# CaNS-World/CaLES

Measured on AMD Instinct MI355X. Metric: time-steps/sec, higher is better.
Workload: dtype f64; 1 GPU; turbulent channel 512x512x512, sgstype=dsmag, PP/PP/NN pressure BCs, bulk forcing in x (BASELINE.json configs[2]); 3 RK substeps/step; decomposition=single GPU

## Files before the change

cales_amd/csrc/common.hpp:

```cpp
#pragma once
#include <hip/hip_runtime.h>
#include <cstdint>
#include <cstdio>
#include <cstdlib>
#include <cstring>
#include <cmath>
#include <string>
#include <vector>
#include "../../include/cales.h"

typedef cales_real real;
#ifdef CALES_SINGLE
typedef float2 real2;
#define CALES_EPS 1.1920929e-07f
#define CALES_BIG 3.4028235e38f
#else
typedef double2 real2;
#define CALES_EPS 2.220446049250313e-16
#define CALES_BIG 1.7976931348623157e308
#endif
constexpr int RSZ = (int)sizeof(real);
constexpr int LINE_REALS = 128 / RSZ;
__host__ __device__ inline real2 make_real2(real x, real y) { real2 r; r.x = x; r.y = y; return r; }

// ... 13 lines not shown
  __host__ __device__ inline real at(int i, int j, int n1) const {
    const real bcv = bc[i + (size_t)(n1 + 2) * j];
    real r = 0.;
    if (cf == 'c') { if (ctype == 'D') r = -2. * bcv / dlc / dlf; else if (ctype == 'N') r = sgn * bcv / dlf; }
    else           { if (ctype == 'D') r = -bcv / dlc / dlf;      else if (ctype == 'N') r = sgn * bcv / dlc; }
    return r * alpha;
  }
};

struct Comm {
  cales_halo_cb halo = nullptr; cales_alltoall_cb a2a = nullptr; cales_allreduce_cb allred = nullptr; void *user = nullptr;
  real *A = nullptr, *B = nullptr; int64_t nbuf = 0;
  bool on = false;
  cales_halo_s_cb halo_s = nullptr; cales_alltoall_part_cb a2a_part = nullptr;
  bool halo_second_stream = false, a2a_second_stream = false, has_lo = false, has_hi = false;
};

struct Spec {
  int blocked, cw, n2l, n3;
  int nyq = 0;
  __host__ __device__ inline size_t at_slab(const Geom &g, int m, int jl, int k) const {
    if (!blocked) return (g.ix(0, jl, k) >> 1) + (size_t)m;
    const int peer = m / cw, mm = m - peer * cw;
    return (size_t)mm + (size_t)cw * ((size_t)(jl - 1) + (size_t)n2l * ((size_t)(k - 1) + (size_t)n3 * peer));
  }
  __host__ __device__ inline size_t at_mode(const Geom &g, int mm, int j, int k) const {
    if (!blocked) return (g.ix(0, j, k) >> 1) + (size_t)mm;
    const int peer = (j - 1) / n2l, jl = (j - 1) - peer * n2l;
    return (size_t)mm + (size_t)cw * ((size_t)jl + (size_t)n2l * ((size_t)(k - 1) + (size_t)n3 * peer));
  }
};

struct Flags {
  bool unfolded_correc = false, unfolded_mom = false, eager_projection = false, lazy_projection = false, helmholtz_z_per_column = false, unfused_imp_rhs = false, unfused_correc = false, unfused_forcing = false, unfused_fillps = false, unfused_mean = false, keep_last_rhs = false, wide_offsets = false, dsmag_reference_sequence = false, dsmag_xghosts = false, smag_reference_sequence = false, gaussel_march = false, fft_generic = false, fft_no_odd_radix = false, keep_null_mode = false, unfused_rk = false, overlap = false, xghosts_in_step = false, unmerged_bc = false, no_nyquist_packing = false, sgs_six_components = false;
  int kchunk = 0; long tile_min_blocks = 2048;
  std::string test_bad_launch;
  void read_env() {
    test_bad_launch = getenv("CALES_TEST_BAD_LAUNCH") ? getenv("CALES_TEST_BAD_LAUNCH") : "";
    unfolded_mom = getenv("CALES_UNFOLDED_MOM") != nullptr;
    lazy_projection = getenv("CALES_LAZY_PROJECTION") != nullptr;
    eager_projection = getenv("CALES_EAGER_PROJECTION") != nullptr;
    unfolded_correc = getenv("CALES_UNFOLDED_CORREC") != nullptr;
    helmholtz_z_per_column = getenv("CALES_HELMHOLTZ_Z_PER_COLUMN") != nullptr;
    unfused_imp_rhs = getenv("CALES_UNFUSED_IMP_RHS") != nullptr;
    unfused_correc = getenv("CALES_UNFUSED_CORREC") != nullptr;
    unfused_forcing = getenv("CALES_UNFUSED_FORCING") != nullptr;
    unfused_fillps = getenv("CALES_UNFUSED_FILLPS") != nullptr;
    unfused_mean = getenv("CALES_UNFUSED_MEAN") != nullptr;
    keep_last_rhs = getenv("CALES_KEEP_LAST_RHS") != nullptr;
    wide_offsets = getenv("CALES_WIDE_OFFSETS") != nullptr;
    dsmag_reference_sequence = getenv("CALES_DSMAG_REFERENCE_SEQUENCE") != nullptr;
    dsmag_xghosts = getenv("CALES_DSMAG_XGHOSTS") != nullptr;
    sgs_six_components = getenv("CALES_SGS_SIX_COMPONENTS") != nullptr;
    smag_reference_sequence = getenv("CALES_SMAG_REFERENCE_SEQUENCE") != nullptr;
    gaussel_march = getenv("CALES_GAUSSEL_MARCH") != nullptr;
    no_nyquist_packing = getenv("CALES_NO_NYQUIST_PACKING") != nullptr;
    fft_generic = getenv("CALES_FFT_GENERIC") != nullptr;
    fft_no_odd_radix = getenv("CALES_FFT_NO_ODD_RADIX") != nullptr;
    xghosts_in_step = getenv("CALES_XGHOSTS_IN_STEP") != nullptr;
    keep_null_mode = getenv("CALES_KEEP_NULL_MODE") != nullptr;
    unfused_rk = getenv("CALES_UNFUSED_RK") != nullptr;
    overlap = getenv("CALES_OVERLAP") != nullptr && atoi(getenv("CALES_OVERLAP")) != 0 && getenv("CALES_NO_OVERLAP") == nullptr;
    unmerged_bc = getenv("CALES_UNMERGED_BC") != nullptr;
    kchunk = getenv("CALES_KCHUNK") ? atoi(getenv("CALES_KCHUNK")) : 0;
    tile_min_blocks = getenv("CALES_TILE_MIN_BLOCKS") ? atol(getenv("CALES_TILE_MIN_BLOCKS")) : 2048;
  }
};

struct StepPlan {
  bool valid = false;
  bool in_visct_zero = false, in_sgs_first = false;
  bool xskip = false;
  bool fold_correc = false;
  bool fold_rows2 = false;
  bool fold_mom = false;
  bool lazy_last = false;
  bool defer_imp_rhs = false;
  bool any_wm = false, skip_first_wm = false;
  bool fuse_cu = false;
  bool defer_force = false;
  bool fuse_fill = false;
  bool visct_ghosts = false;
  bool keep_last_rhs = false;
  int mean_mask = 0, force_mask = 0;
};

struct BandMap { int gx, gy, gz, sub; };
struct TileGeom { dim3 block, grid; int kchunk = 0; BandMap bm{0, 0, 0, 0}; };
// ... 362 lines not shown
```

cales_amd/csrc/k_solver.hip:

```cpp
#include "common.hpp"

struct __attribute__((aligned(2 * sizeof(real)))) cpx { real x, y; };
__device__ inline cpx cadd(cpx a, cpx b) { return {a.x + b.x, a.y + b.y}; }
__device__ inline cpx csub(cpx a, cpx b) { return {a.x - b.x, a.y - b.y}; }
__device__ inline cpx cmul(cpx a, cpx b) { return {a.x * b.x - a.y * b.y, a.x * b.y + a.y * b.x}; }
__device__ inline cpx cconj(cpx a) { return {a.x, -a.y}; }
template <int INV> __device__ inline cpx mul_mi(cpx a) { return INV ? cpx{-a.y, a.x} : cpx{a.y, -a.x}; }

template <int R, int INV>
__device__ inline void fft_stage(const cpx *__restrict__ in, cpx *__restrict__ out, int N, int Ns, int t, int T, const cpx *__restrict__ tw) {
  const int M = N / R, tstep = N / (Ns * R);
  for (int j = t; j < M; j += T) {
    const int k = j % Ns;
    cpx v[R];
#pragma unroll
    for (int r = 0; r < R; ++r) v[r] = in[j + r * M];
    if (Ns > 1) {
#pragma unroll
      for (int r = 1; r < R; ++r) { cpx w = tw[k * r * tstep]; if (INV) w.y = -w.y; v[r] = cmul(v[r], w); }
    }
    const int j0 = (j - k) * R + k;
    if (R == 2) {
      out[j0] = cadd(v[0], v[1]); out[j0 + Ns] = csub(v[0], v[1]);
    } else if (R == 4) {
// ... 1118 lines not shown
      if (ch == 0) sp = 0.;
      real xv = rprev[q] - V[M - 2] * sp - cp[M - 2] * s;
      real mine = (rL == M - 2) ? xv : s;
      col[q * P + M - 2] = xv;
#pragma unroll
      for (int r = M - 3; r >= 0; --r) { xv = col[q * P + r] - V[r] * sp - cp[r] * xv; col[q * P + r] = xv; if (PER && r == rL) mine = xv; }
      col[q * P + M - 1] = s;
      if (PER) {
        const real p11 = __shfl(xv, 0, 64), p1n = __shfl(mine, cL, 64);
        const real an = ra[nz - 1], bn = rb_[nz - 1], cn = rc[nz - 1];
        const real den = (bn + lam) + cn * e1 + an * eL + CALES_EPS;
        const real pn = nullc ? 0. : ((pnr[q] - cn * p11) - an * p1n) * (1. / den);
#pragma unroll
        for (int r = 0; r < M - 1; ++r) if (k0 + r < nsys) col[q * P + r] = col[q * P + r] + E[r] * pn;
        if (k0 + M - 1 < nsys) col[q * P + M - 1] = s + Es * pn;
        if (ch == nsys / M) col[q * P + nsys % M] = pn;
      }
    }
  }
  __syncthreads();
  {
    constexpr int W2 = W / 2, KP2 = NT / W2, NQ2 = 64 * M / KP2;
    const int x = 2 * (t % W2), kk = t / W2;
    const bool ok = W * tile + x < ndbl;
    size_t o = base + x + (size_t)kk * kst;
    int kq = kk;
    asm volatile("" : "+v"(o), "+v"(kq));
    const size_t step = (size_t)KP2 * kst;
#pragma unroll
    for (int q = 0; q < NQ2; ++q) {
      const int k = kq + KP2 * q;
      if (ok && k < nz) *reinterpret_cast<real2 *>(p + o) = make_real2(shz[x * P + k + k / M], shz[(x + 1) * P + k + k / M]);
      o += step;
    }
  }
}
template <int M, int HERM>
__global__ __launch_bounds__(256) void k_gaussel_nyq(Geom g, int nz, int N, int nh, real lscale, const real *__restrict__ abc, const real *__restrict__ lamx,
                                                     const real *__restrict__ lamy, real2 *__restrict__ p, int fixnull, Spec S,
                                                     const real *__restrict__ ra = nullptr, const real *__restrict__ rb_ = nullptr, const real *__restrict__ rc = nullptr) {
  extern __shared__ real shz[];
  constexpr int NV = 1, PER = 0, CP = M + 1, P = 64 * CP + GT_PAD, NT = 256;
  constexpr bool TL = false;
  const real *tabl = nullptr;
  const int nsys = nz;
  const int t = threadIdx.x, ky = HERM ? blockIdx.x : 2 * blockIdx.x, kp = HERM ? (N - ky) % N : ky + 1;
  for (int k = t; k < 64 * M; k += NT) {
    real2 z1 = make_real2(0., 0.), z2 = z1;
    if (k < nz) { z1 = p[S.at_mode(g, 0, ky + 1, k + 1)]; z2 = p[S.at_mode(g, 0, kp + 1, k + 1)]; }
    const int o = k + k / M;
    if (HERM) {
      shz[0 * P + o] = 0.5 * (z1.x + z2.x); shz[1 * P + o] = 0.5 * (z1.y - z2.y);
      shz[2 * P + o] = 0.5 * (z1.y + z2.y); shz[3 * P + o] = -0.5 * (z1.x - z2.x);
    } else { shz[0 * P + o] = z1.x; shz[1 * P + o] = z1.y; shz[2 * P + o] = z2.x; shz[3 * P + o] = z2.y; }
  }
  __syncthreads();
  const int x = t >> 6, ch = t & 63;
  const bool colok = true;
  if (colok) {
    const real lam = HERM ? (lamx[x < 2 ? 0 : nh] + lamy[ky]) * lscale : (lamx[(x & 1) ? nh : 0] + lamy[x < 2 ? ky : kp]) * lscale;
    const bool nullc = fixnull && lam == 0.;
    real *col = shz + x * P + ch * CP;
    const int k0 = ch * M;
    real cp[M - 1], V[M - 1];
    real cprev = 0., vprev = 0., rprev[NV] = {};
    real pnr[NV] = {}, E[PER ? M - 1 : 1] = {}, eprev = 0.;
// ... 389 lines not shown

enum class XKernel { fft_x8, fft_x4, dst1, fft_x };
enum class YKernel { fft_y16, fft_y8, fft_y8r, fft_y4, dst1, fft_y };
enum class ZKernel { herm, tile, ri, periodic_real, periodic_cpx };
static bool radix8_y(YKernel k) { return k == YKernel::fft_y16 || k == YKernel::fft_y8 || k == YKernel::fft_y8r; }
typedef void (*FftX8)(Geom, int, int, const cpx *, const cpx *, const cpx *, real *, real, Spec, real2 *, FillArgs, long, long);
typedef void (*FftX4)(Geom, FftPlan, int, const cpx *, const cpx *, real *, real, Spec, real2 *);
typedef void (*FftX)(Geom, FftPlan, int, int, const cpx *, const cpx *, const cpx *, real *, real, Spec, real2 *);
typedef void (*Dst1)(Geom, FftPlan, int, const cpx *, real *, real, Spec, real2 *, int, int);
typedef void (*FftY16)(Geom, int, int, const cpx *, const cpx *, Spec, real2 *, int, int);
typedef void (*FftY8)(Geom, int, int, int, const cpx *, const cpx *, Spec, real2 *, int, int);
typedef void (*FftY8r)(Geom, int, int, int, const cpx *, Spec, real2 *, int, int);
typedef void (*FftY4)(Geom, FftPlan, int, int, const cpx *, const cpx *, Spec, real2 *);
typedef void (*FftY)(Geom, FftPlan, int, int, int, const cpx *, const cpx *, Spec, real2 *);
struct XPass {
  XKernel k = XKernel::fft_x;
  union { FftX8 x8[3]; FftX4 x4[2]; FftX x[2]; Dst1 dst1[2]; } fn = {{nullptr, nullptr, nullptr}};
  int threads = 256, rows = 1; size_t lds = 0;
  int odd = 0;
  FftPlan plan;
  const cpx *tw = nullptr, *twp = nullptr, *twd = nullptr;
};
struct YPass {
  YKernel k = YKernel::fft_y;
  union { FftY16 y16[2]; FftY8 y8[2]; FftY8r y8r[2]; FftY4 y4[2]; FftY y[2]; Dst1 dst1[2]; } fn = {{nullptr, nullptr}};
  int threads = 256, cols = 1; size_t lds = 0;
  int odd = 0;
  FftPlan plan;
  const cpx *tw = nullptr, *twd = nullptr;
};
constexpr int tile_m(int nz) { return nz <= 128 ? 2 : nz <= 256 ? 4 : nz <= 512 ? 8 : 16; }
static bool tile_takes(const cales_ctx *c, int nz, bool periodic) { return nz >= (periodic ? 4 : 2) && nz <= 1024 && !c->fl.gaussel_march; }
constexpr int TILE_TAB = 3 * 64 * 16;
struct ZTile { int M = 0, NV = 0, PER = 0, DUD = 0, ndbl = 0, nrow = 0; bool persistent = false; real *tab = nullptr; };
struct SolvePath {
  int xkind = 0, ykind = 0;
  XPass xp; YPass yp; ZKernel zk = ZKernel::ri;
  int nz = 0; bool periodic_z = false, poisson = false;
  ZTile zt;
  int fixnull = 0;
  bool refnull = false;
  bool null_switch = false;
  bool nyq = false;
  int cw = 0;
  real *lamx = nullptr, *lamy = nullptr; real normfft = 1.;
};
struct SolveSched {
  real2 *slab_spec = nullptr, *mode_spec = nullptr;
  int nch = 1, kpc = 0; long rows = 0;
  unsigned xblk_f = 0, xblk_b = 0; int xit_f = 1, xit_b = 1, ykc = 1;
  int ncol = 0, ncol_y = 0, mofs = 0, nmodes = 0;
  int64_t a2a_stride = 0, a2a_chunk = 0; int npart = 0;
  Spec S; TileMap T{}; dim3 gz;
};
static real2 *spec_of(real2 *staged, real *pp) { return staged ? staged : reinterpret_cast<real2 *>(pp + 1); }
enum class HzForm { thomas_periodic, thomas_per_column, tile, cols };
struct HzPath {
  HzForm form = HzForm::cols; int nz = 0, q = 0; ZTile zt; TileMap T{};
  real alpha[4] = {0., 0., 0., 0.}; bool ok[4] = {false, false, false, false}; int next = 0;
};
struct Solver {
  real *twx = nullptr, *twx_post = nullptr, *twy = nullptr, *twy_post = nullptr, *twyd = nullptr;
  real *tw4x = nullptr, *tw4y = nullptr, *twy4 = nullptr;
  SolvePath pres, vel[3]; SolveSched sched_pres, sched_vel[3];
  real *d_mpart = nullptr;
  int vel_state[3] = {0, 0, 0}; std::string vel_err[3];
  HzPath hz[3];
  real *d_a = nullptr, *d_b, *d_c, *d_av[3] = {nullptr, nullptr, nullptr}, *d_bv[3], *d_cv[3];
  real *d_scaled = nullptr;
  real *tab_pres = nullptr, *tab_imp3d = nullptr, *tab_hz = nullptr;
  real *d_nullw = nullptr;
};
struct ScaledAbc { real *a, *b, *c, *zz, *dd; };
static ScaledAbc scaled_abc(const cales_ctx *c) { real *p = c->solver->d_scaled; const int n3 = c->n[2]; return {p, p + n3, p + 2 * n3, p + 3 * n3, p + 4 * n3}; }
typedef void (*TileKernel)(Geom, int, int, real, const real *, const real *, const real *, real *, int, TileMap, const real *, const real *, const real *);
static TileKernel tile_kernel(const ZTile &Z) {
#define TILE(M, NV, PER, DUD) case 1000 * M + 100 * NV + 10 * PER + DUD: return k_gaussel_tile<M, NV, PER, DUD>
  switch (1000 * Z.M + 100 * Z.NV + 10 * Z.PER + Z.DUD) {
  TILE(2, 1, 0, 0); TILE(4, 1, 0, 0); TILE(8, 1, 0, 0); TILE(16, 1, 0, 0);
  TILE(2, 2, 0, 0); TILE(4, 2, 0, 0); TILE(8, 2, 0, 0); TILE(16, 2, 0, 0);
  TILE(2, 1, 1, 0); TILE(4, 1, 1, 0); TILE(8, 1, 1, 0); TILE(16, 1, 1, 0);
  TILE(2, 2, 1, 0); TILE(4, 2, 1, 0); TILE(8, 2, 1, 0); TILE(16, 2, 1, 0);
  TILE(2, 2, 0, 1); TILE(4, 2, 0, 1); TILE(8, 2, 0, 1);
  default: return nullptr;
  }
#undef TILE
}
static int tile_lds(int M) { return 16 * (64 * (M + 1) + GT_PAD) * 8 + (GT_TL && M == 16 ? 2 * 64 * M * 8 : 0); }
static void tile_attr(cales_ctx *c, const ZTile &Z) { HIPSOFT(c, hipFuncSetAttribute(Z.persistent ? (const void *)k_gaussel_tile_p<1> : (const void *)tile_kernel(Z), hipFuncAttributeMaxDynamicSharedMemorySize, tile_lds(Z.M))); }
static void tile_table(cales_ctx *c, int M, int nsys, const real *da, const real *db, const real *dc, real *tab) { LAUNCH(c, k_abc_chunked, dim3((64 * M + 255) / 256), dim3(256), 0, c->stream, nsys, M, da, db, dc, tab); }
static void launch_tile(cales_ctx *c, const ZTile &Z, int nz, real lscale, const real *ra, const real *rb_, const real *rc, const real *lamx, const real *lamy, real *p, int fixnull, const TileMap &T) {
  if (Z.persistent) {
    const int ntile = Z.ndbl / 16; int tpb = 1; while (tpb * 2 <= ntile && tpb < 32 && (long)Z.nrow * ((ntile + 2 * tpb - 1) / (2 * tpb)) >= 2048) tpb *= 2;
    LAUNCH(c, (k_gaussel_tile_p<1>), dim3((ntile + tpb - 1) / tpb, Z.nrow), dim3(512), tile_lds(16), c->stream, c->g, nz, Z.ndbl, lscale, Z.tab, lamx, lamy, p, fixnull, T, tpb, ra, rb_, rc);
    return;
  }
  const TileKernel k_gaussel_tile_form = tile_kernel(Z);
  LAUNCH(c, k_gaussel_tile_form, dim3((Z.ndbl + 15) / 16, Z.nrow), dim3(64 * 16 / Z.NV), tile_lds(Z.M), c->stream, c->g, nz, Z.ndbl, lscale, Z.tab, lamx, lamy, p, fixnull, T, ra, rb_, rc);
}
typedef void (*NyqKernel)(Geom, int, int, int, real, const real *, const real *, const real *, real2 *, int, Spec, const real *, const real *, const real *);
static void launch_nyq(cales_ctx *c, const ZTile &Z, bool herm, int nz, int N, int nh, real lscale, const real *lamx, const real *lamy, real2 *p, int fixnull, const Spec &S) {
  static const NyqKernel forms[4][2] = {{k_gaussel_nyq<2, 0>, k_gaussel_nyq<2, 1>}, {k_gaussel_nyq<4, 0>, k_gaussel_nyq<4, 1>}, {k_gaussel_nyq<8, 0>, k_gaussel_nyq<8, 1>}, {k_gaussel_nyq<16, 0>, k_gaussel_nyq<16, 1>}};
  const NyqKernel k_gaussel_nyq_form = forms[Z.M == 2 ? 0 : Z.M == 4 ? 1 : Z.M == 8 ? 2 : 3][herm ? 1 : 0];
  LAUNCH(c, k_gaussel_nyq_form, dim3(herm ? N / 2 + 1 : N / 2), dim3(256), 4 * (64 * (Z.M + 1) + GT_PAD) * 8, c->stream, c->g, nz, N, nh, lscale, Z.tab, lamx, lamy, p, fixnull, S,
         (const real *)nullptr, (const real *)nullptr, (const real *)nullptr);
}
__global__ void k_null_column(Geom, Spec, int, int, const real *, const real *, const real *, const real *, const real *, real2 *, real *, int);
static void launch_z(cales_ctx *c, const SolvePath &P, const SolveSched &D, real *pp, const real *da, const real *db, const real *dc, real lscale) {
  const int n2g = c->C.ng[1], nh = c->C.ng[0] / 2, mh = c->n[0] / 2 + 1, nz = P.nz; real2 *mode_spec = spec_of(D.mode_spec, pp);
  const bool refnull = P.refnull && D.mofs == 0;
  if (refnull) LAUNCH(c, k_null_column, dim3(1), dim3(64), 0, c->stream, c->g, D.S, nz, P.periodic_z ? 1 : 0, da, db, dc, P.lamx, P.lamy, mode_spec, c->solver->d_nullw, 0);
  { ProfScope ps(c, "gaussel_z");
    const dim3 b(64, 4); real *ms = (real *)mode_spec;
    switch (P.zk) {
    case ZKernel::herm:
      LAUNCH(c, k_gaussel_herm, D.gz, dim3(256), 0, c->stream, c->g, nz, D.ncol, n2g, D.mofs, nh, D.S, lscale, da, db, dc, P.lamx, P.lamy, ms, c->scr1, P.fixnull);
      break;
    case ZKernel::tile:
      if (!P.poisson) tile_table(c, P.zt.M, P.zt.PER ? nz - 1 : nz, da, db, dc, P.zt.tab);
      launch_tile(c, P.zt, nz, lscale, da, db, dc, P.lamx, P.lamy, ms, P.fixnull, D.T);
      break;
    case ZKernel::ri:
      LAUNCH(c, k_gaussel_ri, D.gz, dim3(256), 0, c->stream, c->g, nz, D.ncol, n2g, D.mofs, P.xkind ? nh : mh, D.S, lscale, da, db, dc, P.lamx, P.lamy, ms, c->scr1, P.fixnull, P.xkind ? 1 : 0);
      break;
    case ZKernel::periodic_real:
      LAUNCH(c, (k_gaussel<real, 1>), D.gz, b, 0, c->stream, c->g, nz, 2 * nh, n2g, 1, 0, 2 * nh, D.S, lscale, da, db, dc, P.lamx, P.lamy, pp, c->scr1, c->scr2, P.fixnull);
      break;
    case ZKernel::periodic_cpx:
      LAUNCH(c, (k_gaussel<real2, 1>), D.gz, b, 0, c->stream, c->g, nz, D.ncol, n2g, 0, D.mofs, mh, D.S, lscale, da, db, dc, P.lamx, P.lamy, ms, c->scr1, c->scr2, P.fixnull);
      break;
    } }
// ... 98 lines not shown
  if (P.ykind >= 5) {
    Y.k = YKernel::dst1; const int N = dst1_points(P.ykind, n2g); real *tw = nullptr;
    if (N < 2 || !make_plan(N, Y.plan) || (size_t)2 * (N + 1) * sizeof(cpx) > 150 * 1024) { c->err = "helmholtz: y line not supported by the face-centred transform kernel"; return 1; }
    if (upload_twiddles(c, N, N, &tw)) return 1;
    Y.tw = (const cpx *)tw; Y.lds = (size_t)2 * (N + 1) * sizeof(cpx); Y.fn.dst1[0] = Y.fn.dst1[1] = k_dst1<1>; lds_attr(c, Y.fn.dst1, 1, Y.lds); return 0; }
  if (P.ykind >= 3) {
    Y.k = YKernel::fft_y4; if (!make_plan(n2g / 2, Y.plan)) { c->err = std::string(who) + ": ng(2)/2 must factor into primes <= 127"; return 1; }
    Y.lds = stockham_block(4, (size_t)2 * 2 * (n2g / 2 + 1) * sizeof(cpx), &Y.cols);
    if (Y.lds > 64 * 1024) { c->err = std::string(who) + ": y line too long for the LDS-resident DCT-IV"; return 1; }
    if (!s.tw4y && upload_dct4_weights(c, n2g, &s.tw4y)) return 1;
    if (!s.twy4 && upload_twiddles(c, n2g / 2, n2g / 2, &s.twy4)) return 1;
    Y.tw = (const cpx *)s.twy4; Y.twd = (const cpx *)s.tw4y; Y.fn.y4[0] = Y.fn.y4[1] = P.ykind == 3 ? k_fft_y4<0> : k_fft_y4<1>; return 0; }
  Y.k = YKernel::fft_y;
  if (!make_plan(n2g, Y.plan)) { c->err = "solver: ng(1)/2 and ng(2) must factor into primes <= 127"; return 1; }
  Y.lds = stockham_block(8, (size_t)2 * (n2g + 1) * sizeof(cpx), &Y.cols);
  if (Y.lds > 64 * 1024) { c->err = "solver: line too long for the LDS-resident transform"; return 1; }
  Y.fn.y[0] = k_fft_y<0>; Y.fn.y[1] = k_fft_y<1>; return 0;
}
static int choose_kernels(cales_ctx *c, Solver &s, SolvePath &P, const char *who) {
  if (x_pass(c, s, P) || y_pass(c, s, P, who)) return 1;
  const bool hasd = CBP(c, 0, 3) == 'D' || CBP(c, 1, 3) == 'D';
  P.fixnull = (P.poisson && !hasd && !c->fl.keep_null_mode) ? 1 : 0; P.refnull = P.poisson && !hasd && c->fl.keep_null_mode; P.null_switch = c->fl.keep_null_mode;
  if (P.xkind && !P.ykind) P.zk = ZKernel::herm;
  else if ((P.periodic_z || P.fixnull || !P.poisson || hasd) && tile_takes(c, P.nz, P.periodic_z)) P.zk = ZKernel::tile;
  else if (P.xkind) P.zk = P.periodic_z ? ZKernel::periodic_real : ZKernel::ri;
  else P.zk = P.periodic_z ? ZKernel::periodic_cpx : ZKernel::ri;
  return 0;
}
static void tile_setup(cales_ctx *c, SolvePath &P, real *tab) {
  if (P.zk != ZKernel::tile) return;
  ZTile &Z = P.zt; Z.M = tile_m(P.nz); Z.NV = P.xkind ? 1 : 2; Z.PER = P.periodic_z ? 1 : 0; Z.tab = tab;
  Z.ndbl = c->P > 1 ? 2 * P.cw * c->n[1] : P.xkind ? 2 * (c->C.ng[0] / 2) : 2 * (P.nyq ? c->n[0] / 2 : c->n[0] / 2 + 1); Z.nrow = c->P > 1 ? c->P : c->C.ng[1];
  Z.persistent = !Z.PER && Z.NV == 1 && P.nz == 1024 && Z.ndbl % 16 == 0;
  tile_attr(c, Z);
}
static int solve_sched(cales_ctx *c, const SolvePath &P, SolveSched &D) {
  D = SolveSched();
  const int *n = c->n, mh = n[0] / 2 + 1, n2g = c->C.ng[1], nh = c->C.ng[0] / 2, cw = P.cw;
  const bool dist = c->P > 1, use8x = P.xp.k == XKernel::fft_x8, use8y = radix8_y(P.yp.k), use16y = P.yp.k == YKernel::fft_y16;
  const int Rx8 = use8x ? P.xp.rows : 1, CB8 = use8y ? P.yp.cols : 1;
  if (dist) { D.slab_spec = reinterpret_cast<real2 *>(c->comm.A); D.mode_spec = reinterpret_cast<real2 *>(c->comm.B); }
  D.nmodes = P.nyq ? n[0] / 2 : mh; D.ncol = dist ? cw : D.nmodes; D.mofs = dist ? c->rank * cw : 0;
  D.ncol_y = (!dist && P.xkind == 1 && use8y) ? nh : D.ncol;
  D.S.blocked = dist ? 1 : 0; D.S.cw = cw; D.S.n2l = n[1]; D.S.n3 = n[2]; D.S.nyq = P.nyq ? 1 : 0;
  D.T.blocked = dist ? 1 : 0; D.T.cw = cw; D.T.n2l = n[1]; D.T.mofs = D.mofs; D.T.nmode = P.xkind ? nh : D.nmodes; D.T.nyq = P.nyq ? 1 : 0; D.T.kstride = (size_t)2 * cw * n[1]; D.T.segstride = D.T.kstride * n[2];
  D.gz = P.zk == ZKernel::herm ? dim3((unsigned)(((long)4 * D.ncol * (n2g / 2 + 1) + 255) / 256)) : P.zk == ZKernel::ri ? dim3((unsigned)(((long)2 * D.ncol * n2g + 255) / 256))
       : dim3(((P.zk == ZKernel::periodic_real ? 2 * nh : D.ncol) + 63) / 64, (n2g + 3) / 4);
  if (c->comm.a2a_second_stream && use8x && use8y) { if (n[2] % 4 == 0 && n[2] >= 32) D.nch = 4; else if (n[2] % 2 == 0 && n[2] >= 8) D.nch = 2; }
  const bool pipe = D.nch > 1;
  D.kpc = n[2] / D.nch; D.rows = (long)n[1] * D.kpc;
  D.a2a_stride = (int64_t)n[2] * n[1] * cw * 2; D.a2a_chunk = (int64_t)D.kpc * n[1] * cw * 2;
  if (dist && c->P * D.a2a_stride > c->stage.a2a) {
    c->err = "solver: an all-to-all of " + std::to_string(c->P) + " blocks of " + std::to_string(D.a2a_stride) + " reals does not fit the " + std::to_string(c->stage.a2a) + " the staging buffers were sized for";
    return 1;
  }
  const long xgroups = (D.rows + Rx8 - 1) / Rx8;
  int xiters = 1; while (xiters < 8 && xgroups / (xiters * 2) >= 2048 / D.nch) xiters *= 2;
  if (!pipe && xgroups <= 8192) xiters = 1;
  D.xit_f = xiters; D.xit_b = (!pipe && P.xkind == 0 && nh <= 256) ? 1 : xiters;
  D.xblk_f = (unsigned)((xgroups + D.xit_f - 1) / D.xit_f); D.xblk_b = (unsigned)((xgroups + D.xit_b - 1) / D.xit_b); D.npart = (int)(D.xblk_f * D.nch);
  { const long cg = (D.ncol + CB8 - 1) / CB8, from = pipe ? 2048 / D.nch : 8192;
    while (D.ykc < 8 && cg * (D.kpc / (D.ykc * 2)) >= from && D.kpc % (D.ykc * 2) == 0) D.ykc *= 2; }
  if (use16y) {
    const long slots = (long)(c->ncu > 0 ? c->ncu : 256) * (n2g >= 1024 ? 1 : n2g >= 512 ? 2 : 4), tiles = (D.ncol_y + 7) / 8;
    double best = 1e300;
    for (int kc = 1; kc <= 32 && kc <= D.kpc; ++kc) {
// ... 35 lines not shown
  if (choose_kernels(c, s, P, "solver")) return 1;
  { const bool hasd = CBP(c, 0, 3) == 'D' || CBP(c, 1, 3) == 'D';
    P.nyq = P.xkind == 0 && P.ykind <= 1 && P.xp.k == XKernel::fft_x8 && radix8_y(P.yp.k) && !P.periodic_z && (hasd || !c->fl.keep_null_mode) && tile_takes(c, n3, false) && !c->fl.no_nyquist_packing;
    if (P.nyq && P.zk != ZKernel::tile) { c->err = "solver: the packed mode column needs the z solve in the LDS tile"; return 1; }
    P.cw = P.nyq ? (n1 / 2 + c->P - 1) / c->P : c->cw; }
  { double nx, ny;
    if (line_spectrum(c, 0, &c->C.cbcpre[0], false, P.xkind, &P.lamx, &nx) || line_spectrum(c, 1, &c->C.cbcpre[2], false, P.ykind, &P.lamy, &ny)) return 1; P.normfft = 1. / (nx * ny); }
  std::vector<real> abc(3 * (size_t)n3);
  hs_tridmatrix(&c->C.cbcpre[4], n3, c->dzci.data(), c->dzfi.data(), 'c', abc.data(), abc.data() + n3, abc.data() + 2 * n3);
  if (ctx_upload(c, &s.d_a, abc)) return 1;
  s.d_b = s.d_a + n3; s.d_c = s.d_a + 2 * n3;
  if (P.zk == ZKernel::tile) {
    if (ctx_alloc(c, &s.tab_pres, TILE_TAB, false)) return 1;
    tile_setup(c, P, s.tab_pres);
    tile_table(c, P.zt.M, P.zt.PER ? n3 - 1 : n3, s.d_a, s.d_b, s.d_c, s.tab_pres);
  }
  if (P.refnull && ctx_alloc(c, &s.d_nullw, (size_t)5 * (n3 + 2), false)) return 1;
  if (!c->C.impdiff) return 0;
  for (int iv = 0; iv < 3; ++iv) {
    hs_tridmatrix(&c->cbcvel[6 * iv + 4], n3, c->dzci.data(), c->dzfi.data(), iv == 2 ? 'f' : 'c', abc.data(), abc.data() + n3, abc.data() + 2 * n3);
    if (ctx_upload(c, &s.d_av[iv], abc)) return 1;
    s.d_bv[iv] = s.d_av[iv] + n3; s.d_cv[iv] = s.d_av[iv] + 2 * n3;
  }
  if (ctx_alloc(c, &s.d_scaled, (size_t)5 * n3)) return 1;
  if (c->C.impdiff == 1 && ctx_alloc(c, &s.tab_imp3d, TILE_TAB, false)) return 1;
  if (c->C.impdiff != 2) return 0;
  for (int iv = 0; iv < 3; ++iv) {
    HzPath &H = s.hz[iv]; const char *bcz = &c->cbcvel[6 * iv + 4];
    H.q = (iv == 2 && bcz[1] == 'D') ? 1 : 0; H.nz = n3 - H.q;
    H.form = (bcz[0] == 'P' && bcz[1] == 'P') ? HzForm::thomas_periodic : c->fl.helmholtz_z_per_column ? HzForm::thomas_per_column
           : (tile_takes(c, H.nz, false) && H.nz <= 512 && n3 <= 64 * tile_m(H.nz)) ? HzForm::tile : HzForm::cols;
    if (H.form != HzForm::tile) continue;
    H.T.nolam = 1; H.T.nq = n3; H.zt.M = tile_m(H.nz); H.zt.NV = 2; H.zt.ndbl = n[0]; H.zt.nrow = n[1];
    for (int dud = 0; dud <= 1; ++dud) { H.zt.DUD = dud; tile_attr(c, H.zt); }
    if (!s.tab_hz && ctx_alloc(c, &s.tab_hz, (size_t)12 * TILE_TAB, false)) return 1;
  }
  return 0;
}
void solver_teardown(cales_ctx *c) { delete c->solver; c->solver = nullptr; }

__device__ inline real r_add(real a, real b) {
#pragma clang fp contract(off)
  return a + b;
}
__device__ inline real r_mul(real a, real b) {
#pragma clang fp contract(off)
  return a * b;
}
__device__ inline void ref_dgtsv(int n, const real *a, const real *b, const real *c, real *p, real *d) {
#pragma clang fp contract(off)
  const real eps = CALES_EPS;
  real z = (real)1. / r_add(b[0], eps);
  d[0] = r_mul(c[0], z); p[0] = r_mul(p[0], z);
  for (int l = 1; l < n; ++l) {
    z = (real)1. / r_add(r_add(b[l], -r_mul(a[l], d[l - 1])), eps);
    d[l] = r_mul(c[l], z);
    p[l] = r_mul(r_add(p[l], -r_mul(a[l], p[l - 1])), z);
  }
  for (int l = n - 2; l >= 0; --l) p[l] = r_add(p[l], -r_mul(d[l], p[l + 1]));
}
__global__ void k_null_column(Geom g, Spec S, int nz, int periodic, const real *__restrict__ a, const real *__restrict__ b, const real *__restrict__ c,
                              const real *__restrict__ lamx, const real *__restrict__ lamy, real2 *__restrict__ p, real *__restrict__ w, int phase) {
#pragma clang fp contract(off)
  if (threadIdx.x != 0 || blockIdx.x != 0) return;
  const real lam = lamx[0] + lamy[0];
  if (lam != 0.) return;
  real *bb = w, *d = w + nz, *p1 = w + 2 * nz, *p2 = w + 3 * nz, *col = w + 4 * nz;
// ... 151 lines not shown
  p[e0] = v;
  for (int l = 1; l < nz; ++l) { v = (rhs(l) - a[l] * v) * zz[l]; p[e0 + l * st] = v; }
  if (nq > nz) p[e0 + (size_t)nz * st] = rhs(nz);
  for (int l = nz - 2; l >= 0; --l) { v = p[e0 + l * st] - dd[l] * v; p[e0 + l * st] = v; }
}

__global__ void k_scale_abc(int n, real alpha, const real *a, const real *b, const real *c, real *aa, real *bb, real *cc) {
  const int k = blockIdx.x * 64 + threadIdx.x;
  if (k < n) { aa[k] = a[k] * alpha; bb[k] = b[k] * alpha + 1.; cc[k] = c[k] * alpha; }
}
int op_rhs_b_velz(cales_ctx *c, int ivel, real alpha, real *planes = nullptr, int *has = nullptr);
void rhs_b_velz_args(cales_ctx *c, int ivel, real alpha, RhsBz *R, int *has);
int op_rhs_b_velxy(cales_ctx *c, int ivel, real alpha);
int op_helmholtz_z(cales_ctx *c, int ivel, real alpha, bool fused, real hf12) {
  if (c->C.impdiff != 2) { c->err = "helmholtz_z needs impdiff = 2"; return 1; }
  ProfScope ps(c, "helmholtz_z");
  Solver &s = *c->solver; HzPath &H = s.hz[ivel - 1];
  const int *n = c->n; const int n3 = n[2], nz = H.nz; const bool tile = H.form == HzForm::tile;
  int has[2] = {0, 0}; RhsBz RB[2] = {};
  if (fused && tile) rhs_b_velz_args(c, ivel, alpha, RB, has);
  else if (int e = op_rhs_b_velz(c, ivel, alpha, fused ? c->scr2 : nullptr, fused ? has : nullptr)) return e;
  int slot = -1; if (tile) for (int q4 = 0; q4 < 4; ++q4) if (H.ok[q4] && H.alpha[q4] == alpha) slot = q4;
  const bool hit = slot >= 0; if (tile && !hit) { slot = H.next; H.next = (slot + 1) % 4; H.alpha[slot] = alpha; H.ok[slot] = true; }
  const ScaledAbc A = scaled_abc(c);
  if (!hit) LAUNCH(c, k_scale_abc, dim3((n3 + 63) / 64), dim3(64), 0, c->stream, n3, alpha, s.d_av[ivel - 1], s.d_bv[ivel - 1], s.d_cv[ivel - 1], A.a, A.b, A.c);
  const dim3 b(64, 4), gr((n[0] + 63) / 64, (n[1] + 3) / 4);
  real *fld = c->f[CALES_U + ivel - 1];
  const real *dud = c->f[CALES_DUDTD + ivel - 1], *force = c->C.is_forced[ivel - 1] ? c->d_force + (ivel - 1) : nullptr;
  Spec S; S.blocked = 0; S.cw = 0; S.n2l = n[1]; S.n3 = n3;
  switch (H.form) {
  case HzForm::thomas_periodic: LAUNCH(c, (k_gaussel<real, 1>), gr, b, 0, c->stream, c->g, nz, n[0], n[1], 1, 0, n[0], S, 1., A.a, A.b, A.c, (const real *)nullptr, (const real *)nullptr, fld, c->scr1, c->scr2, 0); break;
  case HzForm::thomas_per_column: LAUNCH(c, (k_gaussel<real, 0>), gr, b, 0, c->stream, c->g, nz, n[0], n[1], 1, 0, n[0], S, 1., A.a, A.b, A.c, (const real *)nullptr, (const real *)nullptr, fld, c->scr1, c->scr2, 0); break;
  case HzForm::tile: {
    ZTile Z = H.zt; Z.DUD = fused ? 1 : 0; Z.tab = s.tab_hz + (size_t)(4 * (ivel - 1) + slot) * TILE_TAB; TileMap T = H.T;
    if (fused) { T.dud = dud + 1; T.hf12 = hf12; T.force = force; T.blo = RB[0]; T.bhi = RB[1]; T.has_lo = has[0]; T.has_hi = has[1]; }
    if (!hit) tile_table(c, Z.M, nz, A.a, A.b, A.c, Z.tab);
    launch_tile(c, Z, nz, 1., nullptr, nullptr, nullptr, s.pres.lamx, s.pres.lamy, fld + 1, 0, T);
    break; }
  case HzForm::cols:
    LAUNCH(c, k_thomas_coef, dim3(1), dim3(64), 0, c->stream, nz, A.a, A.b, A.c, A.zz, A.dd);
    if (fused) LAUNCH(c, k_gaussel_cols_rhs, gr, b, 0, c->stream, c->g, nz, n3, A.a, A.zz, A.dd, fld, dud, hf12, force, c->scr2, has[0], has[1]);
    else LAUNCH(c, k_gaussel_cols, gr, b, 0, c->stream, c->g, nz, A.a, A.zz, A.dd, fld);
  }
  LAUNCHCHK(c);
  return 0;
}

static int velocity_path(cales_ctx *c, Solver &s, int iv, SolvePath &V) {
  const int n2g = c->C.ng[1]; const char *bc = &c->cbcvel[6 * iv], *bcz = bc + 4;
  V.xkind = line_kind(bc, iv == 0); V.ykind = line_kind(bc + 2, iv == 1);
  if (V.xkind < 0 || V.ykind < 0) { c->err = "helmholtz: unknown velocity BC pair in x or y"; return 1; }
  if (V.xkind && !V.ykind && bcz[0] == 'P') { c->err = "helmholtz: non-periodic x with periodic y and z is not provided"; return 1; }
  if (V.xkind && bcz[0] == 'P' && c->P > 1) { c->err = "helmholtz: a non-periodic x with periodic z needs one rank"; return 1; }
  if ((V.ykind == 3 || V.ykind == 4) && (n2g % 2)) { c->err = "helmholtz: ND/DN in y need an even ng(2)"; return 1; }
  double nx, ny; if (line_spectrum(c, 0, bc, iv == 0, V.xkind, &V.lamx, &nx) || line_spectrum(c, 1, bc + 2, iv == 1, V.ykind, &V.lamy, &ny)) return 1;
  V.normfft = 1. / (nx * ny);
  V.nz = c->n[2] - ((iv == 2 && bcz[1] == 'D') ? 1 : 0); V.periodic_z = bcz[0] == 'P' && bcz[1] == 'P'; V.poisson = false; V.cw = c->cw;
  if (choose_kernels(c, s, V, "helmholtz")) return 1;
  tile_setup(c, V, s.tab_imp3d);
  return solve_sched(c, V, s.sched_vel[iv]);
}
static int velocity_path_ready(cales_ctx *c, Solver &s, int iv) {
  if (s.vel_state[iv] == 0) { s.vel_state[iv] = velocity_path(c, s, iv, s.vel[iv]) ? 2 : 1; if (s.vel_state[iv] == 2) s.vel_err[iv] = c->err; }
  if (s.vel_state[iv] == 2) { c->err = s.vel_err[iv]; return 1; }
  return 0;
}
std::string helmholtz_path_name(cales_ctx *c, int iv) {
// ... 20 lines not shown
```

Measured before the change: 27.88 time-steps/s.

## Add register-resident tiled z tridiagonal solver replacing LDS transpose variant

Adds a new tiled Gauss elimination kernel for z-direction tridiagonal systems. Each thread keeps its chunk of M rows for two interleaved columns in registers instead of staging the whole column through a padded LDS transpose. Only the per-chunk reduced-system coefficients go through shared memory, where a wavefront-wide parallel cyclic reduction with shuffles solves them before back-substitution in registers. It becomes the default for the two-column, non-periodic, non-fused, non-persistent case, which includes the pressure z-solve. The cost is higher register pressure and a new numerical path that may differ slightly from the old one.

```diff
diff --git a/cales_amd/csrc/common.hpp b/cales_amd/csrc/common.hpp
--- a/cales_amd/csrc/common.hpp
+++ b/cales_amd/csrc/common.hpp
@@ -69,7 +69,7 @@
 };
 
 struct Flags {
-  bool unfolded_correc = false, unfolded_mom = false, eager_projection = false, lazy_projection = false, helmholtz_z_per_column = false, unfused_imp_rhs = false, unfused_correc = false, unfused_forcing = false, unfused_fillps = false, unfused_mean = false, keep_last_rhs = false, wide_offsets = false, dsmag_reference_sequence = false, dsmag_xghosts = false, smag_reference_sequence = false, gaussel_march = false, fft_generic = false, fft_no_odd_radix = false, keep_null_mode = false, unfused_rk = false, overlap = false, xghosts_in_step = false, unmerged_bc = false, no_nyquist_packing = false, sgs_six_components = false;
+  bool unfolded_correc = false, unfolded_mom = false, eager_projection = false, lazy_projection = false, helmholtz_z_per_column = false, unfused_imp_rhs = false, unfused_correc = false, unfused_forcing = false, unfused_fillps = false, unfused_mean = false, keep_last_rhs = false, wide_offsets = false, dsmag_reference_sequence = false, dsmag_xghosts = false, smag_reference_sequence = false, gaussel_march = false, gaussel_lds_transpose = false, fft_generic = false, fft_no_odd_radix = false, keep_null_mode = false, unfused_rk = false, overlap = false, xghosts_in_step = false, unmerged_bc = false, no_nyquist_packing = false, sgs_six_components = false;
   int kchunk = 0; long tile_min_blocks = 2048;
   std::string test_bad_launch;
   void read_env() {
@@ -91,6 +91,7 @@
     sgs_six_components = getenv("CALES_SGS_SIX_COMPONENTS") != nullptr;
     smag_reference_sequence = getenv("CALES_SMAG_REFERENCE_SEQUENCE") != nullptr;
     gaussel_march = getenv("CALES_GAUSSEL_MARCH") != nullptr;
+    gaussel_lds_transpose = getenv("CALES_GAUSSEL_LDS_TRANSPOSE") != nullptr;
     no_nyquist_packing = getenv("CALES_NO_NYQUIST_PACKING") != nullptr;
     fft_generic = getenv("CALES_FFT_GENERIC") != nullptr;
     fft_no_odd_radix = getenv("CALES_FFT_NO_ODD_RADIX") != nullptr;
diff --git a/cales_amd/csrc/k_solver.hip b/cales_amd/csrc/k_solver.hip
--- a/cales_amd/csrc/k_solver.hip
+++ b/cales_amd/csrc/k_solver.hip
@@ -1174,6 +1174,143 @@
       const int k = kq + KP2 * q;
       if (ok && k < nz) *reinterpret_cast<real2 *>(p + o) = make_real2(shz[x * P + k + k / M], shz[(x + 1) * P + k + k / M]);
       o += step;
+    }
+  }
+}
+constexpr int GR_P = 66, GR_F = 8 * GR_P;
+constexpr int gr_park(int M) { return M == 8 ? 4 : 0; }
+__device__ inline bool tile_column2(const TileMap &T, int d, int ndbl, int by, int &mode, int &j) {
+  mode = d >> 1; j = by + 1;
+  bool colok = d < ndbl;
+  if (T.blocked) {
+    const int f = d >> 1, mm = f % T.cw, jl = f / T.cw;
+    j = by * T.n2l + jl + 1;
+    mode = mm + T.mofs;
+    colok = colok && mm + T.mofs < T.nmode;
+  }
+  if (T.nyq && mode == 0) colok = false;
+  return colok;
+}
+template <int M>
+__global__ __launch_bounds__(512, (M <= 8 ? 6 : 2)) void k_gaussel_tile_r(Geom g, int nz, int ndbl, real lscale, const real *__restrict__ abc,
+                                                            const real *__restrict__ lamx, const real *__restrict__ lamy,
+                                                            real *__restrict__ p, int fixnull, TileMap T,
+                                                            const real *__restrict__ = nullptr, const real *__restrict__ = nullptr, const real *__restrict__ = nullptr) {
+  extern __shared__ real shz[];
+  constexpr int W = 16, NPK = gr_park(M);
+  const int lane = threadIdx.x & 63, wv = threadIdx.x >> 6;
+  const int m = lane & 7, ch = 8 * wv + (lane >> 3), k0 = ch * M;
+  const int tile = blockIdx.x;
+  const size_t base = (T.blocked ? T.segstride * blockIdx.y : g.ix(0, blockIdx.y + 1, 1)) + (size_t)W * tile;
+  const size_t kst = T.blocked ? T.kstride : (size_t)g.s12;
+  int mode, j;
+  const bool colok = tile_column2(T, W * tile + 2 * m, ndbl, blockIdx.y, mode, j);
+  real Dv[2][M];
+#pragma unroll
+  for (int r = 0; r < M; ++r) {
+    const int k = k0 + r;
+    const real2 v = (colok && k < nz) ? *reinterpret_cast<const real2 *>(p + base + 2 * m + (size_t)k * kst) : make_real2(0., 0.);
+    Dv[0][r] = v.x; Dv[1][r] = v.y;
+  }
+  real cp[M - 1], V[M - 1];
+  real *sep = shz + m * GR_P + ch, *park = shz + 8 * GR_F + threadIdx.x;
+  if (colok) {
+    const real lam = T.nolam ? 0. : (lamx[mode] + lamy[j - 1]) * lscale;
+    const bool nullc = fixnull && lam == 0.;
+    real cprev = 0., vprev = 0., rprev[2] = {};
+    const real *tb = abc + ch;
+    real An = tb[0], Bn = tb[64 * M], Cn = tb[128 * M];
+#pragma unroll
+    for (int r = 0; r < M - 1; ++r) {
+      const int k = k0 + r;
+      const bool pin = nullc && k == nz - 1, live = k < nz && !pin;
+      const real A0 = An, B0 = Bn, C0 = Cn;
+      An = tb[(r + 1) * 64]; Bn = tb[64 * M + (r + 1) * 64]; if (r + 1 < M - 1) Cn = tb[128 * M + (r + 1) * 64];
+      asm volatile("" ::: "memory");
+      const real A = pin ? 0. : A0, C = pin ? 0. : C0, B = pin ? 1. : B0 + (k < nz ? lam : 0.);
+      const real z = rcp_nr(B - A * cprev + CALES_EPS);
+      cp[r] = C * z; V[r] = (r == 0 ? A : -A * vprev) * z;
+#pragma unroll
+      for (int q = 0; q < 2; ++q) { const real D = live ? Dv[q][r] : 0.; rprev[q] = (D - A * rprev[q]) * z; Dv[q][r] = rprev[q]; }
+      cprev = cp[r]; vprev = V[r];
+    }
+    real Vb = V[M - 2], Wb = cp[M - 2], Rb[2] = {rprev[0], rprev[1]};
+#pragma unroll
+    for (int r = M - 3; r >= 0; --r) {
+      Vb = V[r] - cp[r] * Vb; Wb = -cp[r] * Wb;
+#pragma unroll
+      for (int q = 0; q < 2; ++q) Rb[q] = Dv[q][r] - cp[r] * Rb[q];
+    }
+    {
+      const int k = k0 + M - 1;
+      const bool pin = nullc && k == nz - 1, live = k < nz && !pin;
+      const real A0 = An, B0 = Bn;
+      const real A = pin ? 0. : A0, B = pin ? 1. : B0 + (k < nz ? lam : 0.);
+      sep[0] = -A * V[M - 2]; sep[GR_F] = B - A * cp[M - 2];
+#pragma unroll
+      for (int q = 0; q < 2; ++q) { const real D = live ? Dv[q][M - 1] : 0.; sep[(2 + q) * GR_F] = D - A * rprev[q]; }
+    }
+    sep[4 * GR_F] = Vb; sep[5 * GR_F] = Wb; sep[6 * GR_F] = Rb[0]; sep[7 * GR_F] = Rb[1];
+#pragma unroll
+    for (int r = 0; r < NPK; ++r) park[r * 512] = V[r];
+  }
+  __syncthreads();
+  {
+    int mode2, j2;
+    if (tile_column2(T, W * tile + 2 * wv, ndbl, blockIdx.y, mode2, j2)) {
+      const int ch = lane;
+      real *row = shz + wv * GR_P + ch;
+      const real lam = T.nolam ? 0. : (lamx[mode2] + lamy[j2 - 1]) * lscale;
+      const bool nullc = fixnull && lam == 0., last = ch == 63;
+      const bool pin = nullc && ch * M + M - 1 == nz - 1;
+      const real C0 = abc[128 * M + (M - 1) * 64 + ch], C = pin ? 0. : C0;
+      real al = row[0], be = row[GR_F], ga, de[2] = {row[2 * GR_F], row[3 * GR_F]};
+      real Vn = row[4 * GR_F + 1], Wn = row[5 * GR_F + 1], Rn[2] = {row[6 * GR_F + 1], row[7 * GR_F + 1]};
+      if (last) { Vn = 0.; Wn = 0.; Rn[0] = 0.; Rn[1] = 0.; }
+      be = be - C * Vn; ga = -C * Wn;
+#pragma unroll
+      for (int q = 0; q < 2; ++q) de[q] = de[q] - C * Rn[q];
+#pragma unroll
+      for (int h = 1; h < 64; h <<= 1) {
+        const bool lo = ch >= h, hi = ch + h < 64;
+        const real rb = rcp_nr(be);
+        const real rbm = __shfl_up(rb, h, 64), rbp = __shfl_down(rb, h, 64);
+        const real k1 = lo ? al * rbm : 0., k2 = hi ? ga * rbp : 0.;
+        const real alm = __shfl_up(al, h, 64), gam = __shfl_up(ga, h, 64), alp = __shfl_down(al, h, 64), gap = __shfl_down(ga, h, 64);
+        be = be - gam * k1 - alp * k2;
+#pragma unroll
+        for (int q = 0; q < 2; ++q) de[q] = de[q] - __shfl_up(de[q], h, 64) * k1 - __shfl_down(de[q], h, 64) * k2;
+        al = -alm * k1; ga = -gap * k2;
+      }
+      const real rb = rcp_nr(be);
+#pragma unroll
+      for (int q = 0; q < 2; ++q) row[(2 + q) * GR_F] = de[q] * rb;
+    }
+  }
+  __syncthreads();
+  if (colok) {
+    int t3 = threadIdx.x;
+    asm volatile("" : "+v"(t3));
+    const int m = t3 & 7, ch = 8 * (t3 >> 6) + ((t3 & 63) >> 3);
+    const real *sep = shz + m * GR_P + ch, *park = shz + 8 * GR_F + t3;
+#pragma unroll
+    for (int r = 0; r < NPK; ++r) V[r] = park[r * 512];
+    real *o = p + base + 2 * m + (size_t)(ch * M) * kst;
+#pragma unroll
+    for (int q = 0; q < 2; ++q) {
+      const real s = sep[(2 + q) * GR_F];
+      real sp = sep[(2 + q) * GR_F - (ch > 0 ? 1 : 0)];
+      if (ch == 0) sp = 0.;
+      real xv = Dv[q][M - 2] - V[M - 2] * sp - cp[M - 2] * s;
+      Dv[q][M - 2] = xv;
+#pragma unroll
+      for (int r = M - 3; r >= 0; --r) { xv = Dv[q][r] - V[r] * sp - cp[r] * xv; Dv[q][r] = xv; }
+      Dv[q][M - 1] = s;
+    }
+#pragma unroll
+    for (int r = 0; r < M; ++r) {
+      if (ch * M + r < nz) *reinterpret_cast<real2 *>(o) = make_real2(Dv[0][r], Dv[1][r]);
+      o += kst;
     }
   }
 }
@@ -1629,7 +1766,8 @@
 constexpr int tile_m(int nz) { return nz <= 128 ? 2 : nz <= 256 ? 4 : nz <= 512 ? 8 : 16; }
 static bool tile_takes(const cales_ctx *c, int nz, bool periodic) { return nz >= (periodic ? 4 : 2) && nz <= 1024 && !c->fl.gaussel_march; }
 constexpr int TILE_TAB = 3 * 64 * 16;
-struct ZTile { int M = 0, NV = 0, PER = 0, DUD = 0, ndbl = 0, nrow = 0; bool persistent = false; real *tab = nullptr; };
+struct ZTile { int M = 0, NV = 0, PER = 0, DUD = 0, ndbl = 0, nrow = 0; bool persistent = false; real *tab = nullptr; bool regs = false; };
+static bool tile_form(const cales_ctx *c, const ZTile &Z) { return Z.NV == 2 && !Z.PER && !Z.DUD && !Z.persistent && !c->fl.gaussel_lds_transpose; }
 struct SolvePath {
   int xkind = 0, ykind = 0;
   XPass xp; YPass yp; ZKernel zk = ZKernel::ri;
@@ -1672,6 +1810,7 @@
 static ScaledAbc scaled_abc(const cales_ctx *c) { real *p = c->solver->d_scaled; const int n3 = c->n[2]; return {p, p + n3, p + 2 * n3, p + 3 * n3, p + 4 * n3}; }
 typedef void (*TileKernel)(Geom, int, int, real, const real *, const real *, const real *, real *, int, TileMap, const real *, const real *, const real *);
 static TileKernel tile_kernel(const ZTile &Z) {
+  if (Z.regs) switch (Z.M) { case 2: return k_gaussel_tile_r<2>; case 4: return k_gaussel_tile_r<4>; case 8: return k_gaussel_tile_r<8>; case 16: return k_gaussel_tile_r<16>; default: return nullptr; }
 #define TILE(M, NV, PER, DUD) case 1000 * M + 100 * NV + 10 * PER + DUD: return k_gaussel_tile<M, NV, PER, DUD>
   switch (1000 * Z.M + 100 * Z.NV + 10 * Z.PER + Z.DUD) {
   TILE(2, 1, 0, 0); TILE(4, 1, 0, 0); TILE(8, 1, 0, 0); TILE(16, 1, 0, 0);
@@ -1684,7 +1823,8 @@
 #undef TILE
 }
 static int tile_lds(int M) { return 16 * (64 * (M + 1) + GT_PAD) * 8 + (GT_TL && M == 16 ? 2 * 64 * M * 8 : 0); }
-static void tile_attr(cales_ctx *c, const ZTile &Z) { HIPSOFT(c, hipFuncSetAttribute(Z.persistent ? (const void *)k_gaussel_tile_p<1> : (const void *)tile_kernel(Z), hipFuncAttributeMaxDynamicSharedMemorySize, tile_lds(Z.M))); }
+static int tile_lds(const ZTile &Z) { return Z.regs ? (8 * GR_F + gr_park(Z.M) * 512) * 8 : tile_lds(Z.M); }
+static void tile_attr(cales_ctx *c, const ZTile &Z) { HIPSOFT(c, hipFuncSetAttribute(Z.persistent ? (const void *)k_gaussel_tile_p<1> : (const void *)tile_kernel(Z), hipFuncAttributeMaxDynamicSharedMemorySize, Z.persistent ? tile_lds(16) : tile_lds(Z))); }
 static void tile_table(cales_ctx *c, int M, int nsys, const real *da, const real *db, const real *dc, real *tab) { LAUNCH(c, k_abc_chunked, dim3((64 * M + 255) / 256), dim3(256), 0, c->stream, nsys, M, da, db, dc, tab); }
 static void launch_tile(cales_ctx *c, const ZTile &Z, int nz, real lscale, const real *ra, const real *rb_, const real *rc, const real *lamx, const real *lamy, real *p, int fixnull, const TileMap &T) {
   if (Z.persistent) {
@@ -1693,7 +1833,7 @@
     return;
   }
   const TileKernel k_gaussel_tile_form = tile_kernel(Z);
-  LAUNCH(c, k_gaussel_tile_form, dim3((Z.ndbl + 15) / 16, Z.nrow), dim3(64 * 16 / Z.NV), tile_lds(Z.M), c->stream, c->g, nz, Z.ndbl, lscale, Z.tab, lamx, lamy, p, fixnull, T, ra, rb_, rc);
+  LAUNCH(c, k_gaussel_tile_form, dim3((Z.ndbl + 15) / 16, Z.nrow), dim3(64 * 16 / Z.NV), tile_lds(Z), c->stream, c->g, nz, Z.ndbl, lscale, Z.tab, lamx, lamy, p, fixnull, T, ra, rb_, rc);
 }
 typedef void (*NyqKernel)(Geom, int, int, int, real, const real *, const real *, const real *, real2 *, int, Spec, const real *, const real *, const real *);
 static void launch_nyq(cales_ctx *c, const ZTile &Z, bool herm, int nz, int N, int nh, real lscale, const real *lamx, const real *lamy, real2 *p, int fixnull, const Spec &S) {
@@ -1858,6 +1998,7 @@
   ZTile &Z = P.zt; Z.M = tile_m(P.nz); Z.NV = P.xkind ? 1 : 2; Z.PER = P.periodic_z ? 1 : 0; Z.tab = tab;
   Z.ndbl = c->P > 1 ? 2 * P.cw * c->n[1] : P.xkind ? 2 * (c->C.ng[0] / 2) : 2 * (P.nyq ? c->n[0] / 2 : c->n[0] / 2 + 1); Z.nrow = c->P > 1 ? c->P : c->C.ng[1];
   Z.persistent = !Z.PER && Z.NV == 1 && P.nz == 1024 && Z.ndbl % 16 == 0;
+  Z.regs = tile_form(c, Z);
   tile_attr(c, Z);
 }
 static int solve_sched(cales_ctx *c, const SolvePath &P, SolveSched &D) {
@@ -1959,7 +2100,7 @@
            : (tile_takes(c, H.nz, false) && H.nz <= 512 && n3 <= 64 * tile_m(H.nz)) ? HzForm::tile : HzForm::cols;
     if (H.form != HzForm::tile) continue;
     H.T.nolam = 1; H.T.nq = n3; H.zt.M = tile_m(H.nz); H.zt.NV = 2; H.zt.ndbl = n[0]; H.zt.nrow = n[1];
-    for (int dud = 0; dud <= 1; ++dud) { H.zt.DUD = dud; tile_attr(c, H.zt); }
+    for (int dud = 0; dud <= 1; ++dud) { H.zt.DUD = dud; H.zt.regs = tile_form(c, H.zt); tile_attr(c, H.zt); }
     if (!s.tab_hz && ctx_alloc(c, &s.tab_hz, (size_t)12 * TILE_TAB, false)) return 1;
   }
   return 0;
@@ -2177,7 +2318,7 @@
   case HzForm::thomas_periodic: LAUNCH(c, (k_gaussel<real, 1>), gr, b, 0, c->stream, c->g, nz, n[0], n[1], 1, 0, n[0], S, 1., A.a, A.b, A.c, (const real *)nullptr, (const real *)nullptr, fld, c->scr1, c->scr2, 0); break;
   case HzForm::thomas_per_column: LAUNCH(c, (k_gaussel<real, 0>), gr, b, 0, c->stream, c->g, nz, n[0], n[1], 1, 0, n[0], S, 1., A.a, A.b, A.c, (const real *)nullptr, (const real *)nullptr, fld, c->scr1, c->scr2, 0); break;
   case HzForm::tile: {
-    ZTile Z = H.zt; Z.DUD = fused ? 1 : 0; Z.tab = s.tab_hz + (size_t)(4 * (ivel - 1) + slot) * TILE_TAB; TileMap T = H.T;
+    ZTile Z = H.zt; Z.DUD = fused ? 1 : 0; Z.regs = tile_form(c, Z); Z.tab = s.tab_hz + (size_t)(4 * (ivel - 1) + slot) * TILE_TAB; TileMap T = H.T;
     if (fused) { T.dud = dud + 1; T.hf12 = hf12; T.force = force; T.blo = RB[0]; T.bhi = RB[1]; T.has_lo = has[0]; T.has_hi = has[1]; }
     if (!hit) tile_table(c, Z.M, nz, A.a, A.b, A.c, Z.tab);
     launch_tile(c, Z, nz, 1., nullptr, nullptr, nullptr, s.pres.lamx, s.pres.lamy, fld + 1, 0, T);
```

After: 27.85 time-steps/s. No clear change (-0.1%).
